# nzw0301/SimCLR

Measured on AMD Instinct MI355X. Metric: pretrain images/sec (whole node) + CIFAR-10 linear-probe top-1, ResNet-50, higher is better.
Workload: dtype bf16

## Files before the change

### simclr_amd/csrc/bindings.cpp

```cpp
#include <ATen/core/Tensor.h>
#include <ATen/ops/empty.h>
#include <ATen/ops/zeros.h>
#include <ATen/hip/HIPContext.h>
#include <c10/util/Exception.h>
#include <torch/library.h>

#include <algorithm>
#include <vector>

#include "kernels.h"

using at::Tensor;

namespace {

hipStream_t cur_stream() { return at::hip::getCurrentHIPStream().stream(); }

void check_dev(const Tensor& t, at::ScalarType dt, const char* name) {
  TORCH_CHECK(t.is_cuda(), name, ": expected a GPU tensor");
  TORCH_CHECK(t.scalar_type() == dt, name, ": expected dtype ", dt, " got ", t.scalar_type());
  TORCH_CHECK(t.is_contiguous(), name, ": expected a contiguous tensor");
}

const uint16_t* bf(const Tensor& t, const char* n) {
// ... 345 lines not shown
  if (a3 != nullptr) {
    TORCH_CHECK(A3->numel() == G.numel() && cf != nullptr && coef->numel() >= 3 * S * CO,
                "conv1x1_bwd_dual: lazy BN-backward needs A3 [M][Co] and coef [3][S][Co]");
  }
  conv1x1_bwd_dual(bf(G, "G"), a3, cf, bf(X, "X"), xs, xm,
                   bf(Wt, "Wt"), bfw(gm, "gm"), f32w(stats, "stats"), f32w(wpart, "wpart"),
                   (int)M, (int)CO, (int)CI, (int)S, (int)bps, cur_stream(), xr, dual8);
}

void conv1x1_bwd_dual_s2_op(const Tensor& G, const c10::optional<Tensor>& A3,
                            const c10::optional<Tensor>& coef, const Tensor& X, const Tensor& Wt,
                            const Tensor& gm, const Tensor& wpart, int64_t S, int64_t bps) {
  TORCH_CHECK(X.dim() == 4 && gm.dim() == 4, "conv1x1_bwd_dual_s2: NHWC 4-D X and gm");
  const int64_t N = X.size(0), H = X.size(1), W = X.size(2), CI = X.size(3);
  const int64_t OH = gm.size(1), OW = gm.size(2);
  TORCH_CHECK(gm.size(0) == N && gm.size(3) == CI && OH == (H + 1) / 2 && OW == (W + 1) / 2,
              "conv1x1_bwd_dual_s2: gm is the stride-2 output map");
  const int64_t Mo = N * OH * OW;
  const int64_t CO = G.numel() / Mo;
  TORCH_CHECK(CO == 512 && CI == 256 && G.numel() == Mo * CO && Wt.numel() == CI * CO,
              "conv1x1_bwd_dual_s2: (Co, Ci) = (512, 256) only");
  TORCH_CHECK(S >= 1 && S <= 2 && N % S == 0 && bps >= 1 && (Mo / S) % (64 * bps) == 0,
              "conv1x1_bwd_dual_s2: every block's rows must lie in one segment");
  TORCH_CHECK(wpart.numel() >= S * bps * CO * CI, "conv1x1_bwd_dual_s2: wpart size");
  TORCH_CHECK(Mo * CO * 2 < (int64_t(1) << 31) && X.numel() * 2 < (int64_t(1) << 31),
              "conv1x1_bwd_dual_s2: 32-bit buffer offsets");
  const uint16_t* a3 = optbf(A3, "A3");
  const float* cf = optf32(coef, "coef");
  TORCH_CHECK(a3 == nullptr && cf == nullptr,
              "conv1x1_bwd_dual_s2: dY must be materialised (no lazy BN-backward form)");
  conv1x1_bwd_dual_s2(bf(G, "G"), a3, cf, bf(X, "X"), bf(Wt, "Wt"), bfw(gm, "gm"),
                      f32w(wpart, "wpart"), (int)Mo, (int)CO, (int)CI, (int)S, (int)bps, (int)H,
                      (int)W, (int)OH, (int)OW, cur_stream());
}

void wgrad_reduce_slabs_op(const Tensor& partial, int64_t splits, const Tensor& out, double beta) {
  const int64_t n = out.numel();
  TORCH_CHECK(n % 4 == 0 && partial.numel() >= splits * n && splits >= 1,
              "wgrad_reduce_slabs: sizes");
  wgrad_reduce_slabs(f32w(partial, "partial"), (int)splits, f32w(out, "out"), (size_t)n,
                     (float)beta, cur_stream());
}

void weight_transform(const Tensor& W, const Tensor& Wt, std::vector<int64_t> p) {
  TORCH_CHECK(p.size() == 10, "weight_transform params");
  const int Co = p[0], KH = p[1], KW = p[2], Ci = p[3], KHs = p[4], KWs = p[5];
  TORCH_CHECK(W.numel() == (int64_t)Co * KH * KW * Ci, "weight_transform: W numel");
  TORCH_CHECK(Wt.numel() == (int64_t)Ci * KHs * KWs * Co, "weight_transform: Wt numel");
  for (int a = 0; a < KHs; ++a) {
    const int kh = (int)p[6] + a * (int)p[7];
    TORCH_CHECK(kh >= 0 && kh < KH, "weight_transform: kh out of range");
  }
  for (int a = 0; a < KWs; ++a) {
    const int kw = (int)p[8] + a * (int)p[9];
    TORCH_CHECK(kw >= 0 && kw < KW, "weight_transform: kw out of range");
  }
  conv_weight_transform(bf(W, "W"), bfw(Wt, "Wt"), Co, KH, KW, Ci, KHs, KWs, p[6], p[7], p[8], p[9],
                        cur_stream());
}

Tensor weight_transform_plan(const std::vector<Tensor>& Ws, const std::vector<Tensor>& Wts,
                             std::vector<int64_t> p) {
  const size_t n = Ws.size();
  TORCH_CHECK(n > 0 && Wts.size() == n && p.size() == 10 * n, "weight_transform_plan sizes");
  Tensor host = at::empty({(int64_t)(n * sizeof(WtDesc) / 8) + 1},
                          at::TensorOptions().dtype(at::kLong));
// ... 853 lines not shown
  m.def("stem_s2d(Tensor img, int creal, int P, Tensor(a!) xs) -> ()", &stem_s2d_op);
  m.def("gemm_sk(Tensor A, Tensor B, Tensor? sc, Tensor? sh, int seg, int KS, Tensor(a!) part, "
        "Tensor? bias, Tensor(b!) out) -> ()", &gemm_sk_op);
  m.def("bn_relu_maxpool(Tensor a, Tensor ss, int S, Tensor(a!) y, Tensor(b!) arg, Tensor(c!) asel, "
        "int K, int Sd, int P) -> ()", &bn_relu_maxpool_op);
  m.def("maxpool_bwd_bn(Tensor gy, Tensor arg, Tensor y, Tensor a, Tensor coef, int S, Tensor(a!) da, "
        "int K, int Sd, int P) -> ()", &maxpool_bwd_bn_op);
  m.def("ce_topk(Tensor logits, Tensor y, float gscale, Tensor(a!) loss, Tensor(b!) rank, Tensor(c!)? dlogits=None) -> ()", &ce_topk_op);
  m.def("class_sums(Tensor X, Tensor y, int NC, Tensor(a!) sums, Tensor(b!) counts) -> ()", &class_sums_op);
  m.def("igemm(Tensor A, Tensor B, Tensor(a!) out, Tensor? bias, Tensor(b!)? stats, int[] geom, Tensor? pro_sc=None, Tensor? pro_sh=None, int pro_seg_rows=0, bool pro_relu=False, int epi_mode=0, Tensor? epi_a=None, Tensor? epi_b=None, int variant=-1, Tensor? epi_ss=None, Tensor? epi_mi=None, int seg_rows=0, int stats_seg_blocks=0, int stats_base=0, Tensor? epi_c=None, Tensor? epi_mask=None, Tensor? epi_c2=None, Tensor? epi_mi2=None, Tensor(c!)? stats2=None, Tensor? pro_d=None, Tensor? A2=None, Tensor? pro_rss=None, Tensor(d!)? pro_out=None, Tensor(e!)? pro_mask=None) -> ()", &igemm);
  m.def("igemm_dual_ok(int v, int[] geom) -> bool", &igemm_dok);
  m.def("igemm_bm(int N) -> int", &igemm_bm);
  m.def("igemm_nvariants() -> int", &igemm_nvariants);
  m.def("igemm_variant_bm(int v) -> int", &igemm_vbm);
  m.def("igemm_variant_bn(int v) -> int", &igemm_vbn);
  m.def("igemm_variant_glds(int v) -> bool", &igemm_vglds);
  m.def("igemm_glds_ok(int[] geom, bool pro, bool bn_bwd_pro) -> bool", &igemm_gldsok);
  m.def("wgrad_nvariants() -> int", &wgrad_nvariants);
  m.def("wgrad_xlin(int mode=-1) -> int", &wgrad_xlin_op);
  m.def("wgrad_variant_glds(int v) -> bool", &wgrad_vglds);
  m.def("igemm_variant_patch(int v) -> bool", [](int64_t v) { return igemm_variant_patch((int)v); });
  m.def("wgrad_variant_area(int v) -> int", [](int64_t v) -> int64_t {
    TORCH_CHECK(v >= 0 && v < wgrad_num_variants(), "wgrad variant out of range");
    return wgrad_variant_area((int)v);
  });
  m.def("igemm_variant_ok(int v, int[] geom, bool pro, bool bn_bwd_pro, int epi_mode=0) -> bool",
        &igemm_vok);
  m.def("wgrad_variant_ok(int v, int[] geom, bool pro, bool dy_pro) -> bool", &wgrad_vok);
  m.def("wgrad_splits(int[] geom, int variant=-1) -> int", &wgrad_nsplit);
  m.def("wgrad_tiles(int[] geom, int variant=-1) -> int", &wgrad_ntiles);
  m.def("conv1x1_bwd_dual_s2(Tensor G, Tensor? A3, Tensor? coef, Tensor X, Tensor Wt, "
        "Tensor(a!) gm, Tensor(b!) wpart, int S, int bps) -> ()", &conv1x1_bwd_dual_s2_op);
  m.def("conv1x1_bwd_dual(Tensor G, Tensor? A3, Tensor? coef, Tensor X, Tensor? xss, Tensor? xmi, Tensor Wt, Tensor(a!) gm, Tensor(b!) stats, Tensor(c!) wpart, int S, int bps, Tensor? Xraw=None, bool dual8=False) -> ()", &conv1x1_bwd_dual_op);
  m.def("wgrad_reduce_slabs(Tensor(a!) partial, int splits, Tensor(b!) out, float beta=0.0) -> ()", &wgrad_reduce_slabs_op);
  m.def("wgrad(Tensor dY, Tensor X, Tensor(a!) partial, Tensor(b!) out, int[] geom, int splits, int creal, float beta, Tensor? pro_sc=None, Tensor? pro_sh=None, int pro_seg_rows=0, bool pro_relu=False, int pro_S=1, int variant=-1, Tensor? dY2=None, Tensor? dp_coef=None, int dp_seg_rows=0, int dp_S=1) -> ()", &wgrad);
  m.def("weight_transform(Tensor W, Tensor(a!) Wt, int[] p) -> ()", &weight_transform);
  m.def("weight_transform_plan(Tensor[] Ws, Tensor[] Wts, int[] p) -> Tensor", &weight_transform_plan);
  m.def("weight_transform_batch(Tensor table, int total_blocks) -> ()", &weight_transform_batch);
  m.def("bn_blocks(int R, int C, int S) -> int", &bn_blocks);
  m.def("bn_stats(Tensor x, int S, Tensor(a!) partial) -> ()", &bn_stats);
  m.def("bn_reduce(Tensor partial, int nblk, int S, int C, Tensor(a!) stats) -> ()", &bn_reduce);
  m.def("bn_finalize(Tensor stats, int S, int C, float count, float eps, float momentum, Tensor(a!)? rm, Tensor(b!)? rv, Tensor(c!) mi, Tensor(d!)? nbt, Tensor? gamma=None, Tensor? beta=None, Tensor(e!)? ss=None) -> ()", &bn_final);
  m.def("ipc_collective(int op, Tensor src, Tensor(a!) dst, Tensor peers, Tensor(b!) arena, int site, Tensor(c!) epoch, Tensor(d!) err, int world, int rank) -> ()", &ipc_collective_op);
  m.def("ipc_coll_blocks() -> int", []() -> int64_t { return IPC_COLL_BLOCKS; });
  m.def("bn_reduce_fused(Tensor partial, int nblk, int S, int C, int mode, Tensor(a!)? stats=None, float count=1.0, float eps=1e-5, float momentum=0.1, Tensor(b!)? rm=None, Tensor(c!)? rv=None, Tensor(d!)? mi=None, Tensor(e!)? nbt=None, Tensor? gamma=None, Tensor? beta=None, Tensor(f!)? ss=None, Tensor(g!)? dgamma=None, Tensor(h!)? dbeta=None, Tensor(i!)? coef=None, int ticket_slot=0, Tensor? ipc_peers=None, Tensor(j!)? ipc_arena=None, int ipc_site=0, Tensor(k!)? ipc_epoch=None, Tensor(l!)? ipc_err=None, int world=1, int rank=0) -> ()", &bn_reduce_fused_op);
  m.def("bn_tickets_init(Tensor like) -> ()", [](const Tensor& like) { (void)tickets_for(like, 0, 0); });
  m.def("bn_apply_ss(Tensor x, Tensor ss, Tensor? res, Tensor? rss, Tensor(a!) y, int S, bool relu, Tensor(b!)? mask=None) -> ()", &bn_apply_ss_op);
  m.def("bn_apply(Tensor x, Tensor? res, Tensor(a!) y, Tensor mi, Tensor? gamma, Tensor? beta, int S, bool relu) -> ()", &bn_apply_op);
  m.def("bn_apply_eval(Tensor x, Tensor? res, Tensor(a!) y, Tensor rm, Tensor rv, Tensor? gamma, Tensor? beta, float eps, bool relu) -> ()", &bn_apply_eval_op);
  m.def("bn_bwd_reduce(Tensor dy, Tensor? y, Tensor x, Tensor mi, int S, bool relu, Tensor(a!) partial) -> ()", &bn_bwd_reduce_op);
  m.def("bn_bwd_finalize(Tensor sums, Tensor mi, Tensor? gamma, int S, int C, float count, Tensor(a!)? dgamma, Tensor(b!)? dbeta, Tensor(c!) coef) -> ()", &bn_bwd_final);
  m.def("bn_bwd_apply(Tensor dy, Tensor? y, Tensor x, Tensor coef, int S, bool relu, Tensor(a!) dx, Tensor(b!)? dres) -> ()", &bn_bwd_apply_op);
  m.def("bn_bwd_apply2(Tensor g, Tensor x1, Tensor coef1, Tensor(a!) dx1, Tensor x2, Tensor coef2, Tensor(b!) dx2, int S) -> ()", &bn_bwd_apply2_op);
  m.def("avgpool_fwd(Tensor x, Tensor(a!) y, int Nb, int HW, int C) -> ()", &avgpool_fwd_op);
  m.def("avgpool_bwd(Tensor dy, Tensor(a!) dx, int Nb, int HW, int C) -> ()", &avgpool_bwd_op);
  m.def("colsum(Tensor x, Tensor(a!) out, float beta) -> ()", &colsum_op);
  m.def("cast_to_bf16(Tensor x, Tensor(a!) y) -> ()", &cast_to_bf16);
  m.def("cast_to_f32(Tensor x, Tensor(a!) y) -> ()", &cast_to_f32);
  m.def("nt_normalize(Tensor z, Tensor(a!) zn, Tensor(b!) inv_norm) -> ()", &nt_normalize);
  m.def("nt_transpose(Tensor x, Tensor(a!) out) -> ()", &nt_transpose);
  m.def("nt_transpose_cols(Tensor x, Tensor(a!) out, int c0) -> ()", &nt_transpose_cols);
  m.def("nt_forward_range(Tensor znT, int R, int col_offset, int n_local, float inv_temp, Tensor(a!) part, int c_lo, int c_hi, int splits, int split_base) -> ()", &nt_forward_range);
  m.def("nt_finish(Tensor part, int R, int splits, Tensor(a!) lse, Tensor(b!) loss) -> ()", &nt_finish);
  m.def("nt_fwd_splits(int R, int C) -> int", &nt_fwd_splits);
  m.def("nt_bwd_splits(int nown, int npart) -> int", &nt_bwd_splits);
  m.def("nt_forward(Tensor znT, int R, int col_offset, int n_local, float inv_temp, Tensor(a!) part, int splits, Tensor(b!) lse, Tensor(c!) loss) -> ()", &nt_forward);
// ... 14 lines not shown
```

### simclr_amd/csrc/conv.hip

```cpp
#include <cstring>
#include "common.h"
#include "kernels.h"

#include <type_traits>
#include <utility>

namespace {

struct IgemmArgs {
  const uint16_t* A;
  const uint16_t* B;
  uint16_t* out;
  const float* bias;
  float* stats;
  int M, N, K;
  int IH, IW, C;
  int OH, OW, KW;
  int ish, isw, dh, dw, ih0, iw0;
  int OHp, OWp, osh, osw, ooh, oow, ldo;
  int direct_out;
  uint32_t a_bytes, b_bytes;
  int nMb, nNb;
  const float* pro_sc;
  const float* pro_sh;
// ... 2869 lines not shown
      for (int i = 0; i < 4; ++i)
        wp[(size_t)(wid * (CO / 8) + fm * 16 + g * 4 + i) * CIT + c0 + fn * 16 + li] =
            accw[fm][fn][i];
  if (PLAIN) return;
#pragma unroll
  for (int off = 1; off < 16; off <<= 1)
#pragma unroll
    for (int fn = 0; fn < NF; ++fn)
#pragma unroll
      for (int r = 0; r < 4; ++r) {
        s1[fn][r] += __shfl_xor(s1[fn][r], off, 64);
        s2[fn][r] += __shfl_xor(s2[fn][r], off, 64);
      }
  if (li == 0) {
#pragma unroll
    for (int fn = 0; fn < NF; ++fn)
#pragma unroll
      for (int r = 0; r < 4; ++r) {
        const int ci = cq * CW + fn * 16 + 4 * g + r;
        red[(rh * CI + ci) * 2 + 0] = s1[fn][r];
        red[(rh * CI + ci) * 2 + 1] = s2[fn][r];
      }
  }
  __syncthreads();
  if (tid < CI) {
    float a = 0.f, b = 0.f;
#pragma unroll
    for (int q = 0; q < RG; ++q) {
      a += red[(q * CI + tid) * 2 + 0];
      b += red[(q * CI + tid) * 2 + 1];
    }
    p.stats[((size_t)blk * 2 + 0) * CIT + c0 + tid] = a;
    p.stats[((size_t)blk * 2 + 1) * CIT + c0 + tid] = b;
  }
}

}

void conv_weight_transform_batch(const WtDesc* d, int n, int total_blocks, hipStream_t s) {
  hipLaunchKernelGGL(weight_transform_batch, dim3(total_blocks), dim3(256), 0, s, d, n);
  HIP_CHECK_LAUNCH();
}

int igemm_num_variants() { return kNumIgemm; }
int igemm_variant_bm(int v) { return IG_VARIANTS[v].bm; }
int igemm_variant_bn(int v) { return IG_VARIANTS[v].bn; }
int igemm_default_variant(int N) { return N <= 64 ? 1 : 0; }
bool igemm_variant_glds(int v) { return v >= 0 && v < kNumIgemm && IG_VARIANTS[v].fam != IG_NT; }
bool igemm_variant_patch(int v) {
  return v >= 0 && v < kNumIgemm && IG_VARIANTS[v].fam == IG_PATCH;
}
bool igemm_glds_ok(const ConvGeom& g, bool pro, bool bn_bwd_pro) {
  if (g.C % 64 != 0) return false;
  return !(pro || bn_bwd_pro) || (g.KH == 1 && g.KW == 1 && g.ih0 == 0 && g.iw0 == 0);
}
static bool direct_out(const ConvGeom& g) {
  return g.osh == 1 && g.osw == 1 && g.ooh == 0 && g.oow == 0 && g.OHp == g.OH && g.OWp == g.OW;
}
bool igemm_patch_ok(const ConvGeom& g) {
  return g.KH == 3 && g.KW == 3 && g.ish == 1 && g.isw == 1 && g.dh == 1 && g.dw == 1 &&
         g.ih0 == -1 && g.iw0 == -1 && g.OH == g.IH && g.OW == g.IW &&
         (g.OW == 16 || g.OW == 32) && (g.C == 64 || g.C == 128) && direct_out(g);
}
static bool glds_doubled_fits(const IgemmVariant& r, const ConvGeom& g, int words) {
  const size_t lds = igemm_glds_pro_offset(r.bm, r.bn, r.threads(), g.C > 64 ? 2 : 1, 2) +
                     (size_t)4 * words * g.C;
// ... 247 lines not shown
  } else if (CO == 256 && CI == 64 && xss == nullptr) {
    hipLaunchKernelGGL((conv1x1_bwd_dual<256, 64, true>), dim3(S * bps), dim3(256), lds, s, a);
  } else if (CO == 256 && CI == 64 && Xraw == nullptr) {
    hipLaunchKernelGGL((conv1x1_bwd_dual<256, 64>), dim3(S * bps), dim3(256), lds, s, a);
  } else {
    fprintf(stderr, "conv1x1_bwd_dual: unsupported Co=%d Ci=%d\n", CO, CI);
    abort();
  }
  HIP_CHECK_LAUNCH();
}

void conv1x1_bwd_dual_s2(const uint16_t* G, const uint16_t* A3, const float* coef,
                         const uint16_t* X, const uint16_t* Wt, uint16_t* gm, float* wpart,
                         int Mo, int CO, int CI, int S, int bps, int H, int W, int OH, int OW,
                         hipStream_t s) {
  Dual1x1Args a{};
  a.G = G; a.A3 = A3; a.coef = coef; a.X = X; a.Wt = Wt; a.gm = gm; a.wpart = wpart;
  a.M = Mo; a.S = S; a.seg_rows = Mo / S; a.bps = bps;
  a.tiles_per_block = a.seg_rows / 32 / bps;
  a.g_bytes = (uint32_t)((size_t)Mo * CO * 2);
  a.x_bytes = (uint32_t)((size_t)(Mo / (OH * OW)) * H * W * CI * 2);
  a.xH = H; a.xW = W; a.xOH = OH; a.xOW = OW;
  if (CO != 512 || CI != 256) {
    fprintf(stderr, "conv1x1_bwd_dual_s2: unsupported Co=%d Ci=%d\n", CO, CI);
    abort();
  }
  const dim3 grid(S * bps * (CI / 64)), blk(512);
  const size_t wl = conv1x1_bwd_dual_w_lds(512);
  hipLaunchKernelGGL((conv1x1_bwd_dual_w<512, 256, false, false, true, true>), grid, blk, wl, s,
                     a);
  HIP_CHECK_LAUNCH();
}

void wgrad_reduce_slabs(float* partial, int splits, float* out, size_t n, float beta,
                        hipStream_t s) {
  reduce_slabs(partial, splits, out, n / 4, beta, true, s);
}
```

### simclr_amd/csrc/kernels.h

```cpp
#pragma once
#include <hip/hip_runtime.h>
#include <stddef.h>
#include <stdint.h>

struct ConvGeom {
  int Nb, IH, IW, C;
  int OH, OW;
  int KH, KW;
  int ish, isw, dh, dw;
  int ih0, iw0;
  int N;
  int OHp, OWp, osh, osw, ooh, oow, ldo;
};

struct ConvFusion {
  const float* pro_sc = nullptr;
  const float* pro_sh = nullptr;
  int pro_seg_rows = 0;
  int pro_relu = 0;
  int pro_S = 1;
  const float* pro_d = nullptr;
  const uint16_t* A2 = nullptr;
  const float* pro_rsc = nullptr;
  const float* pro_rsh = nullptr;
// ... 22 lines not shown
int igemm_num_variants();
int igemm_variant_bm(int v);
int igemm_variant_bn(int v);
int igemm_default_variant(int N);
bool igemm_variant_glds(int v);
bool igemm_variant_patch(int v);
bool igemm_glds_ok(const ConvGeom& g, bool pro, bool bn_bwd_pro);
bool igemm_patch_ok(const ConvGeom& g);
bool igemm_variant_ok(int v, const ConvGeom& g, bool pro, bool bn_bwd_pro, int epi_mode = 0);
bool igemm_dual_ok(int v, const ConvGeom& g);
int igemm_block_m(int N);
void conv_igemm_nt(const ConvGeom& g, const uint16_t* A, size_t a_elems, const uint16_t* B,
                   uint16_t* out, const float* bias, float* stats, const ConvFusion& f,
                   int variant, hipStream_t s);
int wgrad_num_variants();
int wgrad_xlin(int mode);
int wgrad_default_variant(int N);
bool wgrad_variant_glds(int v);
int wgrad_variant_area(int v);
bool wgrad_variant_ok(int v, const ConvGeom& g, bool pro, bool dy_pro);
int wgrad_splits(const ConvGeom& g, int variant);
void conv_wgrad(const ConvGeom& g, const uint16_t* dY, const uint16_t* X, size_t x_elems,
                float* partial, int splits, float* out, int Creal, float beta,
                const ConvFusion& f, int variant, hipStream_t s);
size_t conv1x1_bwd_dual_lds();
void conv1x1_bwd_dual(const uint16_t* G, const uint16_t* A3, const float* coef, const uint16_t* X,
                      const float* xss, const float* xmi, const uint16_t* Wt, uint16_t* gm,
                      float* stats, float* wpart, int M, int CO, int CI, int S, int bps,
                      hipStream_t s, const uint16_t* Xraw = nullptr, bool dual8 = false);
void conv1x1_bwd_dual_s2(const uint16_t* G, const uint16_t* A3, const float* coef,
                         const uint16_t* X, const uint16_t* Wt, uint16_t* gm, float* wpart,
                         int Mo, int CO, int CI, int S, int bps, int H, int W, int OH, int OW,
                         hipStream_t s);
void wgrad_reduce_slabs(float* partial, int splits, float* out, size_t n, float beta,
                        hipStream_t s);
int wgrad_tiles(const ConvGeom& g, int variant);
struct WtDesc {
  const uint16_t* W;
  uint16_t* Wt;
  int Co, KH, KW, Ci, KHs, KWs, kh0, sh, kw0, sw, blk0, nblk;
};
static_assert(sizeof(WtDesc) == 64, "WtDesc layout");
void conv_weight_transform_batch(const WtDesc* d, int n, int total_blocks, hipStream_t s);
void conv_weight_transform(const uint16_t* W, uint16_t* Wt, int Co, int KH, int KW, int Ci,
                           int KHs, int KWs, int kh0, int sh, int kw0, int sw, hipStream_t s);

void bn_stats_partial(const uint16_t* x, int R, int C, int S, float* partial, int* nblk_per_seg,
                      hipStream_t s);
int bn_stats_blocks_per_seg(int R, int C, int S);
int bn_reduce_groups(int nblk);
int bn_reduce_direct_rows();
void bn_reduce_partials(const float* partial, int nblk_per_seg, int S, int C, float* stats,
                        float* ws, hipStream_t s);
void bn_finalize(const float* stats, int S, int C, float count, float eps, float momentum,
                 float* running_mean, float* running_var, float* mean_invstd, int64_t* nbt,
                 const float* gamma, const float* beta, float* scale_shift, hipStream_t s);
struct BnReduceFusedParams {
  const float* partial = nullptr;
  int nblk = 0, S = 1, C = 0, mode = 0;
  float* ws = nullptr;
  unsigned* tickets = nullptr;
  float* stats = nullptr;
  float count = 1.f, eps = 1e-5f, momentum = 0.1f;
  float* running_mean = nullptr;
  float* running_var = nullptr;
  float* mi = nullptr;
// ... 178 lines not shown
```

### simclr_amd/models/fused.py

```python
from __future__ import annotations

import os
from dataclasses import dataclass, field
from typing import List, NamedTuple, Optional, Tuple, Union

import torch
import torch.distributed as dist

from ..ops import _ext
from ..ops.conv_hip import (BlockOut, BnApply, BnBackward, Epilogue, Igemm, StatsOut, WgradDY,
                            WgradX, DgradLaunch, dgrad_plan, fwd_geom, run_wgrad, shadow_ohwi,
                            wt_shape)
from ..parallel import state as pstate
from ..parallel.state import site_key


_SKIP_WGRAD = os.environ.get("SIMCLR_SKIP_WGRAD", "0") == "1"
_SKIP_BNRED = os.environ.get("SIMCLR_EXPERIMENT_SKIP_BNREDUCE", "")


def _empty_nhwc(n, h, w, c, dev, dtype=torch.bfloat16):
    return torch.empty((n, h, w, c), device=dev, dtype=dtype)


# ... 208 lines not shown

class _OutGrad(NamedTuple):
    g3: torch.Tensor
    da: torch.Tensor
    lazy: Optional[LazyBN]
    dad: Optional[torch.Tensor]
    ds_dual: Optional[tuple]


class FusedStages:

    BLOCK_OUT_PROLOGUE = True
    STEM_FUSED = os.environ.get("SIMCLR_FUSED_STEM", "1") != "0"

    bnb_prologue = True
    _bnb_max_cin = 128
    lazy_bn1 = False
    mat_expand_min_cin = 128
    lazy_bn3_ds = True
    _lazy_bn3_ds_dual_only = True
    patch_bnb = os.environ.get("SIMCLR_PATCH_BNB", "1") != "0"
    wgrad_stream = os.environ.get("SIMCLR_WGRAD_STREAM", "1") != "0"
    branch_stream = os.environ.get("SIMCLR_BRANCH_STREAM", "1") != "0"
    compact_ds = True
    block_out_min_hw = 1
    block_out_prologue = BLOCK_OUT_PROLOGUE
    fused_bwd1x1 = True
    fused_bwd1x1_wide = True
    dual8 = True
    dual_reduce_main = False
    fused_ds_dual = True
    ds_dual_stream = "main"
    fused_ds_dual_s2 = False
    bwd1x1_bps = _BWD1X1_BPS
    bwd1x1_bps_wide = 64
    stem_s2d = True

    _side = _branch = _wt_event = _s2d_cache = _wt_sig = _wt_table = None
    _wt_ready = False
    stem = _stem_block = stem_pool = None

    def __init__(self, resnet: torch.nn.Module, segments: int = 2):
        from .resnet import BasicBlock, Bottleneck
        self.resnet = resnet
        self.S = segments
        self.calls = 0
        self.dual_launches = 0
        self.out_apply_calls = 0
        self._side_keep: List[torch.Tensor] = []
        self._wt_cache = {}
        self._dual_cache = {}
        self._patch_bnb_cache = {}
        self.block_out_prologue = type(self).BLOCK_OUT_PROLOGUE
        for kv in filter(None, os.environ.get("SIMCLR_FUSED_ATTRS", "").split(",")):
            k, v = kv.split("=", 1)
            if not hasattr(self, k):
                raise ValueError(f"SIMCLR_FUSED_ATTRS: FusedStages has no switch {k!r}")
            if v.lower() in ("true", "false"):
                setattr(self, k, v.lower() == "true")
            else:
                try:
                    setattr(self, k, int(v))
                except ValueError:
                    setattr(self, k, v)
        self.stem_fused = type(self).STEM_FUSED
        from .resnet import _Identity
        from ..ops.pooling import MaxPool2d
        mp = getattr(resnet, "maxpool", None)
# ... 144 lines not shown

    def _bn_bwd(self, ops, bn, partial, nblk_seg: int, bs: _BNState, S: int, st) -> torch.Tensor:
        return self._bn_bwd_finish(ops, self._bn_bwd_start(ops, bn, partial, nblk_seg, bs, S, st),
                                   S)

    def _memo(self, name: str) -> dict:
        if name not in vars(self):
            setattr(self, name, {})
        return vars(self)[name]

    def _side_stream(self, dev) -> "torch.cuda.Stream":
        if self._side is None or self._side.device != dev:
            self._side = torch.cuda.Stream(device=dev)
        return self._side

    def _issue_wgrad(self, cs: _ConvSpec, keep, compute, main: bool = False) -> None:
        if _SKIP_WGRAD:
            compute = lambda out: None
        side = self._side if self.wgrad_stream and not main else None
        if side is None:
            _deliver_grad(cs.conv.weight, compute)
            return
        self._side_keep.extend(keep)
        side.wait_stream(torch.cuda.current_stream(keep[0].device))
        with torch.cuda.stream(side):
            _deliver_grad(cs.conv.weight, compute)

    def _reduce_slabs(self, ops, cs: _ConvSpec, wpart: torch.Tensor, nslab: int) -> None:
        self._issue_wgrad(cs, (wpart,), lambda out: ops.wgrad_reduce_slabs(wpart, nslab, out),
                          main=self.dual_reduce_main)

    def _wgrad(self, ops, dyn, xn, cs: _ConvSpec, pro_ss: Optional[torch.Tensor], S: int,
               bnb: Optional[LazyBN] = None, main: bool = False):
        Nb, H, W, C = xn.shape
        Co = cs.conv.out_channels
        OH, OW = dyn.shape[1], dyn.shape[2]
        s2d = pro_ss is None and self._s2d_ok(cs, xn)
        if s2d:
            xn = self._s2d_input(ops, xn)
            g = fwd_geom(Nb, xn.shape[1], xn.shape[2], 16, OH, OW, 4, 4, 1, 0, Co)
        else:
            g = fwd_geom(Nb, H, W, C, OH, OW, cs.k, cs.k, cs.stride, cs.pad, Co)
        M = Nb * OH * OW
        pro = WgradX(pro_ss[0], pro_ss[1], M // S, True, S) if pro_ss is not None else None
        dpro = WgradDY(*bnb, M // S, S) if bnb is not None else None

        concurrent = bool(self.wgrad_stream) and self._side is not None and not main

        def compute(out):
            if s2d:
                gs = torch.empty((Co, 4, 4, 16), device=dyn.device, dtype=torch.float32)
                run_wgrad(ops, dyn, xn, gs, g, 16, pro=pro, dpro=dpro, concurrent=concurrent)
                self._s2d_unfold_grad(gs, out)
            else:
                run_wgrad(ops, dyn, xn, out, g, cs.conv.in_channels, pro=pro, dpro=dpro,
                          concurrent=concurrent)

        self._issue_wgrad(cs, [t for t in (dyn, xn, pro_ss, *(bnb or ())) if t is not None],
                          compute, main)

    @staticmethod
    def _bwd1x1_bps(rows_seg: int, cap: int = _BWD1X1_BPS) -> int:
        tiles = rows_seg // 64
        b = min(cap, tiles)
        while b > 1 and tiles % b:
            b -= 1
# ... 89 lines not shown
        return cs.k == 1 and cout >= 4 * cin and cin >= self.mat_expand_min_cin

    def _lazy_bn3_ds_ok(self, b: _BlockSpec, tp: _BlockTape, aL: torch.Tensor, S: int) -> bool:
        L = len(b.convs) - 1
        if not (self.lazy_bn3_ds and L > 0 and self._bnb_ok(b.convs[L], aL, S)):
            return False
        if not self._lazy_bn3_ds_dual_only:
            return True
        xin, pro_ss = tp.ins[L]
        return self._bwd1x1_ok(b.convs[L], aL, xin, pro_ss, tp.acts[L - 1], S)

    def _patch_bnb_ok(self, ops, cs: _ConvSpec, a: torch.Tensor, S: int) -> bool:
        if not (self.patch_bnb and a.is_cuda and cs.k == 3 and cs.stride == 1 and cs.pad == 1):
            return False
        Nb, H, W, C = a.shape
        M = Nb * H * W
        if M % S or (M // S) % 256:
            return False
        Ci = cs.conv.in_channels
        key = (Nb, H, W, C, Ci)
        cache = self._memo("_patch_bnb_cache")
        if key not in cache:
            g = dgrad_plan(Nb, H, W, Ci, H, W, C, 3, 1, 1).launches[0].geom
            cache[key] = any(ops.igemm_variant_patch(v) and ops.igemm_variant_ok(v, g, True, True)
                             for v in range(ops.igemm_nvariants()))
        return cache[key]

    def _lazy_bn1_ok(self, b: _BlockSpec, a1: torch.Tensor, S: int) -> bool:
        cs0 = b.convs[0]
        M = a1.numel() // a1.shape[-1]
        return (self.lazy_bn1 and cs0.k == 1 and cs0.stride == 1
                and M % S == 0 and (M // S) % 256 == 0)

    def _dgrad(self, ops, dyn, cs: _ConvSpec, in_shape, S: int, accumulate: bool = False,
               dx: Optional[torch.Tensor] = None,
               bn_epi: Union[None, MaskEpi, ResEpi] = None, bnb: Optional[LazyBN] = None,
               compact: bool = False, sub_resid: bool = False,
               bnb_out: Optional[torch.Tensor] = None):
        Nb, H, W, Ci = in_shape
        _, OH, OW, Co = dyn.shape
        dev = dyn.device
        if bn_epi is not None:
            bn_epi = (MaskEpi if bn_epi[0] == "mask" else ResEpi)._make(bn_epi)
        w = shadow_ohwi(cs.conv.weight, Ci)
        plan = dgrad_plan(Nb, H, W, Ci, OH, OW, Co, cs.k, cs.stride, cs.pad, compact)
        launches = [(self._dgrad_weight(ops, cs, w, ln), ln) for ln in plan.launches]
        if compact:
            assert bn_epi is None and not accumulate
            dc = _empty_nhwc(Nb, OH, OW, Ci, dev)
            (wt, ln), = launches
            job = Igemm(dyn, wt, dc, ln.geom)
            job.launch(ops, job.choose(ops))
            return dc, None, 0
        resid_c = None
        if sub_resid:
            assert cs.stride == 1 and (accumulate or bn_epi is not None)
            resid_c = dx if bn_epi is None else bn_epi.resid
            dx = None
        if dx is None:
            dx = _empty_nhwc(Nb, H, W, Ci, dev)
        if plan.zero_fill:
            assert bn_epi is None, "BN-epilogue dgrad needs every output position covered"
            if not accumulate:
                dx.zero_()
        if bn_epi is None:
            epi = Epilogue(1, dx) if accumulate else None
            if resid_c is not None:
                epi = Epilogue(1, resid_c, sub=True)
            for wt, ln in launches:
                job = Igemm(dyn, wt, dx, ln.geom, epi=epi)
                job.launch(ops, job.choose(ops))
            return dx, None, 0
        assert not accumulate
        if bn_epi.kind == "mask":
            bs = bn_epi.bs
            epi = Epilogue(3, b=bn_epi.a_prev, ss=bs.ss.view(-1), mi=bs.mi)
# ... 356 lines not shown
    def _chain_bwd(self, ops, st, S, b: _BlockSpec, tp: _BlockTape, o: _OutGrad, prev):
        L = len(b.convs) - 1
        g3, da, lazy = o.g3, o.da, o.lazy
        lazy0 = None
        pend = None
        for i in range(L, 0, -1):
            cs = b.convs[i]
            xin, pro_ss = tp.ins[i]
            a_prev, bs_prev = tp.acts[i - 1], tp.bns[i - 1]
            _ext.TAG = f"{b.name} conv{i + 1} dgrad"
            dyn, bnb = (g3, lazy) if (i == L and lazy is not None) else (da, None)
            if pend is not None:
                gsrc, lazy_b = pend
                pend = None
                dy_m = torch.empty_like(lazy_b.a)
                gm, part, nb = self._dgrad(ops, gsrc, cs, a_prev.shape, S,
                                           bn_epi=MaskEpi("mask", a_prev, bs_prev),
                                           bnb=lazy_b, bnb_out=dy_m)
                wdy, wbnb = dy_m, None
            elif self._bwd1x1_ok(cs, dyn, xin, pro_ss, a_prev, S):
                _ext.TAG = f"{b.name} conv{i + 1} dgrad+wgrad"
                gm, part, nb = self._bwd1x1_fused(ops, dyn, bnb, cs, a_prev, bs_prev, S, xin)
                wdy = None
            else:
                gm, part, nb = self._dgrad(ops, dyn, cs, a_prev.shape, S,
                                           bn_epi=MaskEpi("mask", a_prev, bs_prev), bnb=bnb)
                wdy, wbnb = dyn, bnb
            h = self._bn_bwd_start(ops, b.convs[i - 1].bn, part, nb, bs_prev, S, st)
            if wdy is not None:
                _ext.TAG = f"{b.name} conv{i + 1} wgrad"
                self._wgrad(ops, wdy, xin, cs, pro_ss, S, bnb=wbnb)
            _ext.TAG = f"{b.name} bn{i} bwd"
            coef = self._bn_bwd_finish(ops, h, S)
            if i == 1 and prev is not None and self._lazy_bn1_ok(b, a_prev, S):
                lazy0 = LazyBN(a_prev, coef)
                da = gm
                continue
            if i - 1 >= 1 and self._patch_bnb_ok(ops, b.convs[i - 1], a_prev, S):
                pend = (gm, LazyBN(a_prev, coef))
                continue
            da_next = torch.empty_like(a_prev)
            ops.bn_bwd_apply(gm, None, a_prev, coef, S, False, da_next, None)
            da = da_next
        return da, lazy0

    def _conv1_dgrad(self, ops, st, S, b: _BlockSpec, tp: _BlockTape, o: _OutGrad, da, lazy0,
                     resid, join, compact: bool, prev):
        cs0 = b.convs[0]
        if b.down is None:
            resid = o.g3
        elif join is not None:
            torch.cuda.current_stream(tp.ad.device).wait_stream(join)
        elif resid is None:
            _ext.TAG = f"{b.name} ds dgrad"
            resid, _, _ = self._dgrad(ops, o.dad, b.down, tp.x.shape, S, compact=compact)
        _ext.TAG = f"{b.name} conv1 dgrad"
        if prev is None:
            dx, _, _ = self._dgrad(ops, da, cs0, tp.x.shape, S, accumulate=True, dx=resid,
                                   sub_resid=compact)
            return dx, None
        pb, ptp = prev
        pds = pb.down is not None
        dx, part, nb = self._dgrad(ops, da, cs0, tp.x.shape, S, bnb=lazy0,
                                   dx=resid if b.down is not None and not compact else None,
                                   sub_resid=compact,
                                   bn_epi=ResEpi("res", resid, ptp.mask, ptp.acts[-1],
                                                 ptp.bns[-1].mi, ptp.ad if pds else None,
# ... 36 lines not shown
```

Baseline: 24830.

## Fuse conv1 BN-backward, dgrad, wgrad and next BN stats into one kernel

Adds a fused kernel for the first 1x1 conv of non-downsampling bottleneck blocks. It applies the lazy BN-backward to dY, computes dgrad and wgrad partials from the same LDS tile, and in its epilogue adds the residual, applies the ReLU mask and accumulates the previous BN's backward statistics (optionally for two BN streams). The Python side routes conv1 dgrad to it and defers the wgrad to a slab reduction. This removes several separate passes over dY, X and the residual, at the cost of a large single-occupancy kernel with heavy LDS use.

```diff
diff --git a/simclr_amd/csrc/bindings.cpp b/simclr_amd/csrc/bindings.cpp
--- a/simclr_amd/csrc/bindings.cpp
+++ b/simclr_amd/csrc/bindings.cpp
@@ -401,6 +401,58 @@
   conv1x1_bwd_dual_s2(bf(G, "G"), a3, cf, bf(X, "X"), bf(Wt, "Wt"), bfw(gm, "gm"),
                       f32w(wpart, "wpart"), (int)Mo, (int)CO, (int)CI, (int)S, (int)bps, (int)H,
                       (int)W, (int)OH, (int)OW, cur_stream());
+}
+
+void conv1_bwd_dual_op(const Tensor& G, const Tensor& A1, const Tensor& coef, const Tensor& X,
+                       const Tensor& Wt, const Tensor& res, const Tensor& mask, const Tensor& c1,
+                       const Tensor& mi1, const c10::optional<Tensor>& c2,
+                       const c10::optional<Tensor>& mi2, const Tensor& gm, const Tensor& stats,
+                       const c10::optional<Tensor>& stats2, const Tensor& wpart, int64_t S,
+                       int64_t bps) {
+  const int64_t CI = gm.size(-1);
+  const int64_t M = gm.numel() / CI;
+  TORCH_CHECK(M > 0 && G.numel() % M == 0, "conv1_bwd_dual: G rows");
+  const int64_t CO = G.numel() / M;
+  TORCH_CHECK((CO == 64 || CO == 128) && (CI == 256 || CI == 512),
+              "conv1_bwd_dual: Co 64 | 128 and Ci 256 | 512");
+  const int64_t bmt = conv1_bwd_dual_tile((int)CO);
+  TORCH_CHECK(S >= 1 && bps >= 1 && M % S == 0 && (M / S) % 64 == 0 &&
+                  (M / S) % (bmt * bps) == 0,
+              "conv1_bwd_dual: whole 64-row tiles per segment, equal tile shares per block");
+  TORCH_CHECK(A1.numel() == M * CO && X.numel() == M * CI && Wt.numel() == CI * CO &&
+                  res.numel() == M * CI && c1.numel() == M * CI,
+              "conv1_bwd_dual: operand sizes");
+  TORCH_CHECK(coef.numel() >= 3 * S * CO && mi1.numel() >= 2 * S * CI,
+              "conv1_bwd_dual: coef [3][S][Co], mi [2][S][Ci]");
+  check_dev(mask, at::kByte, "mask");
+  TORCH_CHECK(mask.numel() * 8 >= M * CI, "conv1_bwd_dual: mask size");
+  TORCH_CHECK(stats.numel() >= S * bps * 2 * CI && wpart.numel() >= S * bps * CO * CI,
+              "conv1_bwd_dual: stats / wpart size");
+  TORCH_CHECK(M * CI * 2 < (int64_t(1) << 31), "conv1_bwd_dual: 32-bit buffer offsets");
+  const uint16_t* c2p = optbf(c2, "c2");
+  const float* mi2p = optf32(mi2, "mi2");
+  float* st2 = optf32w(stats2, "stats2");
+  TORCH_CHECK((c2p != nullptr) == (mi2p != nullptr) && (c2p != nullptr) == (st2 != nullptr),
+              "conv1_bwd_dual: c2, mi2 and stats2 together");
+  if (c2p != nullptr)
+    TORCH_CHECK(c2->numel() == M * CI && mi2->numel() >= 2 * S * CI &&
+                    stats2->numel() >= S * bps * 2 * CI,
+                "conv1_bwd_dual: second BN stream sizes");
+  TORCH_CHECK(gm.data_ptr() != X.data_ptr() && gm.data_ptr() != c1.data_ptr() &&
+                  (c2p == nullptr || gm.data_ptr() != c2->data_ptr()),
+              "conv1_bwd_dual: gm must not alias X or the x-hat sources");
+  conv1_bwd_dual(bf(G, "G"), bf(A1, "A1"), f32(coef, "coef"), bf(X, "X"), bf(Wt, "Wt"),
+                 bf(res, "res"), mask.data_ptr<uint8_t>(), bf(c1, "c1"), f32(mi1, "mi1"), c2p,
+                 mi2p, bfw(gm, "gm"), f32w(stats, "stats"), st2, f32w(wpart, "wpart"), (int)M,
+                 (int)CO, (int)CI, (int)S, (int)bps, cur_stream());
+}
+
+bool conv1_bwd_dual_ok_op(std::vector<int64_t> gv, int64_t S) {
+  TORCH_CHECK(gv.size() == 22, "conv geometry must have 22 entries");
+  ConvGeom g;
+  int* p = &g.Nb;
+  for (int i = 0; i < 22; ++i) p[i] = (int)gv[i];
+  return conv1_bwd_dual_ok(g, (int)S);
 }
 
 void wgrad_reduce_slabs_op(const Tensor& partial, int64_t splits, const Tensor& out, double beta) {
@@ -1320,6 +1372,13 @@
   m.def("conv1x1_bwd_dual_s2(Tensor G, Tensor? A3, Tensor? coef, Tensor X, Tensor Wt, "
         "Tensor(a!) gm, Tensor(b!) wpart, int S, int bps) -> ()", &conv1x1_bwd_dual_s2_op);
   m.def("conv1x1_bwd_dual(Tensor G, Tensor? A3, Tensor? coef, Tensor X, Tensor? xss, Tensor? xmi, Tensor Wt, Tensor(a!) gm, Tensor(b!) stats, Tensor(c!) wpart, int S, int bps, Tensor? Xraw=None, bool dual8=False) -> ()", &conv1x1_bwd_dual_op);
+  m.def("conv1_bwd_dual(Tensor G, Tensor A1, Tensor coef, Tensor X, Tensor Wt, Tensor res, "
+        "Tensor mask, Tensor c1, Tensor mi1, Tensor? c2, Tensor? mi2, Tensor(a!) gm, "
+        "Tensor(b!) stats, Tensor(c!)? stats2, Tensor(d!) wpart, int S, int bps) -> ()",
+        &conv1_bwd_dual_op);
+  m.def("conv1_bwd_dual_ok(int[] geom, int S) -> bool", &conv1_bwd_dual_ok_op);
+  m.def("conv1_bwd_dual_tile(int Co) -> int",
+        [](int64_t co) -> int64_t { return conv1_bwd_dual_tile((int)co); });
   m.def("wgrad_reduce_slabs(Tensor(a!) partial, int splits, Tensor(b!) out, float beta=0.0) -> ()", &wgrad_reduce_slabs_op);
   m.def("wgrad(Tensor dY, Tensor X, Tensor(a!) partial, Tensor(b!) out, int[] geom, int splits, int creal, float beta, Tensor? pro_sc=None, Tensor? pro_sh=None, int pro_seg_rows=0, bool pro_relu=False, int pro_S=1, int variant=-1, Tensor? dY2=None, Tensor? dp_coef=None, int dp_seg_rows=0, int dp_S=1) -> ()", &wgrad);
   m.def("weight_transform(Tensor W, Tensor(a!) Wt, int[] p) -> ()", &weight_transform);
diff --git a/simclr_amd/csrc/conv.hip b/simclr_amd/csrc/conv.hip
--- a/simclr_amd/csrc/conv.hip
+++ b/simclr_amd/csrc/conv.hip
@@ -2925,6 +2925,262 @@
     }
     p.stats[((size_t)blk * 2 + 0) * CIT + c0 + tid] = a;
     p.stats[((size_t)blk * 2 + 1) * CIT + c0 + tid] = b;
+  }
+}
+
+struct Conv1DualArgs {
+  const uint16_t* G;
+  const uint16_t* A1;
+  const float* coef;
+  const uint16_t* X;
+  const uint16_t* Wt;
+  const uint16_t* res;
+  const uint8_t* mask;
+  const uint16_t* c1;
+  const float* mi1;
+  const uint16_t* c2;
+  const float* mi2;
+  uint16_t* gm;
+  float* stats;
+  float* stats2;
+  float* wpart;
+  int S, seg_rows, bps, tiles_per_block;
+  uint32_t g_bytes, x_bytes;
+};
+
+constexpr int conv1_dual_tile(int CO, bool two = false) { return CO == 64 && !two ? 64 : 32; }
+
+template <int CO>
+__device__ __forceinline__ int conv1_wkey(int r) {
+  if constexpr (CO == 64)
+    return ((r >> 1) & 1) | (((r >> 3) & 1) << 1) | (((r >> 4) & 1) << 2);
+  else
+    return (r & 3) | (((r >> 3) & 3) << 2);
+}
+
+template <int CO, int CIT, bool TWO>
+__global__ __launch_bounds__(512, 1) void conv1_bwd_dual(Conv1DualArgs p) {
+  constexpr int BMT = conv1_dual_tile(CO, TWO);
+  constexpr int CI = 256;
+  constexpr int NH = CIT / CI, NT = 512;
+  constexpr int RF = BMT / 16;
+  constexpr int WM = 2, WN = 4;
+  constexpr int TCO = CO / WM, TKK = CI / WN;
+  static_assert((CO == 64 || CO == 128) && CIT % CI == 0, "conv1 dual tile mappings");
+  static_assert(BMT * (CO / 8) <= NT, "at most one dY chunk per thread and tile");
+  extern __shared__ __attribute__((aligned(16))) char smem[];
+  uint16_t* Ds = (uint16_t*)smem;
+  uint16_t* Xs = Ds + 2 * BMT * CO;
+  uint16_t* Ws = Xs + 2 * BMT * CI;
+  float* Tb = (float*)(Ws + CI * CO);
+  float* Cf = Tb + 4 * CI;
+
+  const int tid = threadIdx.x, lane = tid & 63;
+  const int wid = __builtin_amdgcn_readfirstlane(tid >> 6);
+  const int g = lane >> 4, li = lane & 15;
+  const int lb = xcd_remap(blockIdx.x, gridDim.x);
+  const int half = lb % NH;
+  const int blk = lb / NH;
+  const int c0 = half * CI;
+  const int seg = blk / p.bps;
+  const int mbeg = seg * p.seg_rows + (blk - seg * p.bps) * p.tiles_per_block * BMT;
+  const int T = p.tiles_per_block;
+
+  const __amdgpu_buffer_rsrc_t rg = buf_rsrc(p.G, p.g_bytes);
+  const __amdgpu_buffer_rsrc_t ra = buf_rsrc(p.A1, p.g_bytes);
+  const __amdgpu_buffer_rsrc_t rx = buf_rsrc(p.X, p.x_bytes);
+
+  for (int c = tid; c < CI * CO / 8; c += NT) {
+    const int row = c / (CO / 8), ch = c % (CO / 8);
+    *(u32x4*)(Ws + row * CO + ((ch ^ conv1_wkey<CO>(row)) * 8)) =
+        *(const u32x4*)(p.Wt + ((size_t)(c0 + row) * CO + ch * 8));
+  }
+  for (int i = tid; i < (TWO ? 4 : 2) * CI; i += NT) {
+    const int k = i / CI, c = i % CI;
+    Tb[i] = (k < 2 ? p.mi1 : p.mi2)[((k & 1) * p.S + seg) * CIT + c0 + c];
+  }
+  for (int i = tid; i < 3 * CO; i += NT) {
+    const int k = i / CO, c = i % CO;
+    Cf[i] = p.coef[(k * p.S + seg) * CO + c];
+  }
+
+  constexpr int GCH = CO / 8, XCH = CI / 8;
+  constexpr int XR = NT / XCH;
+  constexpr int XJ = BMT / XR;
+  const int gch = tid % GCH, grow = tid / GCH;
+  const bool gown = BMT * GCH == NT || wid < BMT * GCH / 64;
+  const int xch = tid % XCH, xrow = tid / XCH;
+
+  u32x4 rG[2], rA[2], rX[2][XJ];
+  auto gload = [&](int t, u32x4& G1, u32x4& A1, u32x4 (&X4)[XJ]) {
+    const int m0 = mbeg + t * BMT;
+    const uint32_t off = (uint32_t)(((size_t)(m0 + grow) * CO + gch * 8) * 2);
+    if (gown) {
+      G1 = __builtin_amdgcn_raw_buffer_load_b128(rg, off, 0, 0);
+      A1 = __builtin_amdgcn_raw_buffer_load_b128(ra, off, 0, 0);
+    }
+#pragma unroll
+    for (int j = 0; j < XJ; ++j)
+      X4[j] = __builtin_amdgcn_raw_buffer_load_b128(
+          rx, (uint32_t)(((size_t)(m0 + xrow + XR * j) * CIT + c0 + xch * 8) * 2), 0, 0);
+  };
+  auto lstore = [&](int buf, const u32x4& G1, const u32x4& A1, const u32x4 (&X4)[XJ]) {
+    if (gown)
+      *(u32x4*)(Ds + buf * BMT * CO + grow * CO + tr_swz<CO>(grow, gch * 8)) =
+          bnbwd8(G1, A1, Cf + gch * 8, Cf + CO + gch * 8, Cf + 2 * CO + gch * 8, true);
+#pragma unroll
+    for (int j = 0; j < XJ; ++j) {
+      const int r = xrow + XR * j;
+      *(u32x4*)(Xs + buf * BMT * CI + r * CI + tr_swz<CI>(r, xch * 8)) = X4[j];
+    }
+  };
+
+  struct Epi {
+    u32x4 ea[RF], ec[RF], ec2[RF];
+    unsigned bits[RF];
+  };
+  const int ecol = wid * 32 + 8 * g;
+  auto eload = [&](int t, Epi& e) {
+#pragma unroll
+    for (int rf = 0; rf < RF; ++rf) {
+      const size_t o = (size_t)(mbeg + t * BMT + rf * 16 + li) * CIT + c0 + ecol;
+      e.ea[rf] = __builtin_nontemporal_load((const u32x4*)(p.res + o));
+      e.ec[rf] = __builtin_nontemporal_load((const u32x4*)(p.c1 + o));
+      if (TWO) e.ec2[rf] = *(const u32x4*)(p.c2 + o);
+      e.bits[rf] = p.mask[o >> 3];
+    }
+  };
+
+  f32x4 accw[TCO / 16][TKK / 16];
+#pragma unroll
+  for (int i = 0; i < TCO / 16; ++i)
+#pragma unroll
+    for (int j = 0; j < TKK / 16; ++j) accw[i][j] = (f32x4){0.f, 0.f, 0.f, 0.f};
+  float s1[8], s2[8], s3[8];
+#pragma unroll
+  for (int e = 0; e < 8; ++e) { s1[e] = 0.f; s2[e] = 0.f; s3[e] = 0.f; }
+
+  auto compute = [&](int t, const Epi& ep) {
+    const int cur = t & 1;
+    const uint16_t* Db = Ds + cur * BMT * CO;
+    f32x4 accd[RF][2];
+#pragma unroll
+    for (int rf = 0; rf < RF; ++rf)
+#pragma unroll
+      for (int h = 0; h < 2; ++h) accd[rf][h] = (f32x4){0.f, 0.f, 0.f, 0.f};
+#pragma unroll
+    for (int ks = 0; ks < CO / 32; ++ks) {
+      const int lch = ks * 4 + g;
+      bf16x8 af[2];
+#pragma unroll
+      for (int h = 0; h < 2; ++h) {
+        const int wr = wid * 32 + 8 * (li >> 2) + 4 * h + (li & 3);
+        af[h] = *(const bf16x8*)(Ws + wr * CO + ((lch ^ conv1_wkey<CO>(wr)) * 8));
+      }
+#pragma unroll
+      for (int rf = 0; rf < RF; ++rf) {
+        const int mrow = rf * 16 + li;
+        const bf16x8 bfr = *(const bf16x8*)(Db + mrow * CO + tr_swz<CO>(mrow, lch * 8));
+#pragma unroll
+        for (int h = 0; h < 2; ++h)
+          accd[rf][h] = __builtin_amdgcn_mfma_f32_16x16x32_bf16(af[h], bfr, accd[rf][h], 0, 0, 0);
+      }
+    }
+    wgrad_mma<CO, CI, WM, WN, BMT / 32>(Db, Xs + cur * BMT * CI, accw);
+    float mu[8], in[8], mu2[8], in2[8];
+#pragma unroll
+    for (int e = 0; e < 8; ++e) {
+      mu[e] = Tb[ecol + e];
+      in[e] = Tb[CI + ecol + e];
+      if (TWO) {
+        mu2[e] = Tb[2 * CI + ecol + e];
+        in2[e] = Tb[3 * CI + ecol + e];
+      }
+    }
+#pragma unroll
+    for (int rf = 0; rf < RF; ++rf) {
+      const size_t o = (size_t)(mbeg + t * BMT + rf * 16 + li) * CIT + c0 + ecol;
+      const unsigned bits = ep.bits[rf];
+      u32x4 w;
+#pragma unroll
+      for (int e = 0; e < 4; ++e) {
+        const f32x4& a = accd[rf][e >> 1];
+        const uint32_t dx = pack2bf(a[2 * (e & 1)], a[2 * (e & 1) + 1]);
+        const uint32_t sum =
+            pack2bf(lo_bf(dx) + lo_bf(ep.ea[rf][e]), hi_bf(dx) + hi_bf(ep.ea[rf][e]));
+        const float g0 = (bits >> (2 * e)) & 1u ? lo_bf(sum) : 0.f;
+        const float g1 = (bits >> (2 * e + 1)) & 1u ? hi_bf(sum) : 0.f;
+        w[e] = pack2bf(g0, g1);
+        s1[2 * e] += g0;
+        s2[2 * e] += g0 * ((lo_bf(ep.ec[rf][e]) - mu[2 * e]) * in[2 * e]);
+        s1[2 * e + 1] += g1;
+        s2[2 * e + 1] += g1 * ((hi_bf(ep.ec[rf][e]) - mu[2 * e + 1]) * in[2 * e + 1]);
+        if (TWO) {
+          s3[2 * e] += g0 * ((lo_bf(ep.ec2[rf][e]) - mu2[2 * e]) * in2[2 * e]);
+          s3[2 * e + 1] += g1 * ((hi_bf(ep.ec2[rf][e]) - mu2[2 * e + 1]) * in2[2 * e + 1]);
+        }
+      }
+      __builtin_nontemporal_store(w, (u32x4*)(p.gm + o));
+    }
+  };
+
+  __syncthreads();
+  if (T > 0) {
+    gload(0, rG[0], rA[0], rX[0]);
+    lstore(0, rG[0], rA[0], rX[0]);
+  }
+  if (T > 1) gload(1, rG[1], rA[1], rX[1]);
+  __syncthreads();
+  for (int t = 0; t < T; t += 2) {
+    {
+      Epi ep;
+      eload(t, ep);
+      if (t + 2 < T) gload(t + 2, rG[0], rA[0], rX[0]);
+      compute(t, ep);
+    }
+    if (t + 1 < T) lstore(1, rG[1], rA[1], rX[1]);
+    asm volatile("s_waitcnt lgkmcnt(0)" ::: "memory");
+    __builtin_amdgcn_s_barrier();
+    if (t + 1 >= T) break;
+    {
+      Epi ep;
+      eload(t + 1, ep);
+      if (t + 3 < T) gload(t + 3, rG[1], rA[1], rX[1]);
+      compute(t + 1, ep);
+    }
+    if (t + 2 < T) lstore(0, rG[0], rA[0], rX[0]);
+    asm volatile("s_waitcnt lgkmcnt(0)" ::: "memory");
+    __builtin_amdgcn_s_barrier();
+  }
+  float* wp = p.wpart + (size_t)blk * CO * CIT;
+  const int wm = wid / WN, wn = wid % WN;
+#pragma unroll
+  for (int fm = 0; fm < TCO / 16; ++fm)
+#pragma unroll
+    for (int fn = 0; fn < TKK / 16; ++fn)
+#pragma unroll
+      for (int i = 0; i < 4; ++i)
+        wp[(size_t)(wm * TCO + fm * 16 + g * 4 + i) * CIT + c0 + wn * TKK + fn * 16 + li] =
+            accw[fm][fn][i];
+#pragma unroll
+  for (int off = 1; off < 16; off <<= 1)
+#pragma unroll
+    for (int e = 0; e < 8; ++e) {
+      s1[e] += __shfl_xor(s1[e], off, 64);
+      s2[e] += __shfl_xor(s2[e], off, 64);
+      if (TWO) s3[e] += __shfl_xor(s3[e], off, 64);
+    }
+  if (li == 0) {
+#pragma unroll
+    for (int e = 0; e < 8; ++e) {
+      const size_t c = (size_t)c0 + ecol + e;
+      p.stats[((size_t)blk * 2 + 0) * CIT + c] = s1[e];
+      p.stats[((size_t)blk * 2 + 1) * CIT + c] = s2[e];
+      if (TWO) {
+        p.stats2[((size_t)blk * 2 + 0) * CIT + c] = s1[e];
+        p.stats2[((size_t)blk * 2 + 1) * CIT + c] = s3[e];
+      }
+    }
   }
 }
 
@@ -3238,6 +3494,55 @@
   HIP_CHECK_LAUNCH();
 }
 
+int conv1_bwd_dual_tile(int CO) { return conv1_dual_tile(CO); }
+
+bool conv1_bwd_dual_ok(const ConvGeom& g, int S) {
+  if (!(g.KH == 1 && g.KW == 1 && g.ish == 1 && g.isw == 1 && g.ih0 == 0 && g.iw0 == 0 &&
+        g.OH == g.IH && g.OW == g.IW && direct_out(g)))
+    return false;
+  if (!(g.N == 64 || g.N == 128) || !(g.C == 256 || g.C == 512) || g.C % 64 != 0) return false;
+  if (g.ldo != g.N) return false;
+  const long long M = (long long)g.Nb * g.OH * g.OW;
+  if (S < 1 || M % S != 0 || (M / S) % 64 != 0) return false;
+  return M * g.C * 2 < (1LL << 31);
+}
+
+template <int CO, int CIT>
+static void launch_conv1_dual(const Conv1DualArgs& a, int blocks, hipStream_t s) {
+  const int BMT = conv1_dual_tile(CO, a.c2 != nullptr);
+  const size_t lds = (size_t)2 * BMT * CO * 2 + (size_t)2 * BMT * 256 * 2 + (size_t)256 * CO * 2 +
+                     (size_t)4 * 256 * 4 + (size_t)3 * CO * 4;
+  const dim3 grid(blocks * (CIT / 256)), blk(512);
+  if (a.c2 != nullptr)
+    hipLaunchKernelGGL((conv1_bwd_dual<CO, CIT, true>), grid, blk, lds, s, a);
+  else
+    hipLaunchKernelGGL((conv1_bwd_dual<CO, CIT, false>), grid, blk, lds, s, a);
+}
+
+void conv1_bwd_dual(const uint16_t* G, const uint16_t* A1, const float* coef, const uint16_t* X,
+                    const uint16_t* Wt, const uint16_t* res, const uint8_t* mask,
+                    const uint16_t* c1, const float* mi1, const uint16_t* c2, const float* mi2,
+                    uint16_t* gm, float* stats, float* stats2, float* wpart, int M, int CO,
+                    int CI, int S, int bps, hipStream_t s) {
+  Conv1DualArgs a{};
+  a.G = G; a.A1 = A1; a.coef = coef; a.X = X; a.Wt = Wt; a.res = res; a.mask = mask;
+  a.c1 = c1; a.mi1 = mi1; a.c2 = c2; a.mi2 = mi2; a.gm = gm;
+  a.stats = stats; a.stats2 = stats2; a.wpart = wpart;
+  a.S = S; a.seg_rows = M / S; a.bps = bps;
+  a.tiles_per_block = a.seg_rows / conv1_dual_tile(CO, c2 != nullptr) / bps;
+  a.g_bytes = (uint32_t)((size_t)M * CO * 2);
+  a.x_bytes = (uint32_t)((size_t)M * CI * 2);
+  if (CO == 64 && CI == 256) launch_conv1_dual<64, 256>(a, S * bps, s);
+  else if (CO == 128 && CI == 256) launch_conv1_dual<128, 256>(a, S * bps, s);
+  else if (CO == 64 && CI == 512) launch_conv1_dual<64, 512>(a, S * bps, s);
+  else if (CO == 128 && CI == 512) launch_conv1_dual<128, 512>(a, S * bps, s);
+  else {
+    fprintf(stderr, "conv1_bwd_dual: unsupported Co=%d Ci=%d\n", CO, CI);
+    abort();
+  }
+  HIP_CHECK_LAUNCH();
+}
+
 void wgrad_reduce_slabs(float* partial, int splits, float* out, size_t n, float beta,
                         hipStream_t s) {
   reduce_slabs(partial, splits, out, n / 4, beta, true, s);
diff --git a/simclr_amd/csrc/kernels.h b/simclr_amd/csrc/kernels.h
--- a/simclr_amd/csrc/kernels.h
+++ b/simclr_amd/csrc/kernels.h
@@ -78,6 +78,13 @@
                          const uint16_t* X, const uint16_t* Wt, uint16_t* gm, float* wpart,
                          int Mo, int CO, int CI, int S, int bps, int H, int W, int OH, int OW,
                          hipStream_t s);
+bool conv1_bwd_dual_ok(const ConvGeom& g, int S);
+int conv1_bwd_dual_tile(int CO);
+void conv1_bwd_dual(const uint16_t* G, const uint16_t* A1, const float* coef, const uint16_t* X,
+                    const uint16_t* Wt, const uint16_t* res, const uint8_t* mask,
+                    const uint16_t* c1, const float* mi1, const uint16_t* c2, const float* mi2,
+                    uint16_t* gm, float* stats, float* stats2, float* wpart, int M, int CO,
+                    int CI, int S, int bps, hipStream_t s);
 void wgrad_reduce_slabs(float* partial, int splits, float* out, size_t n, float beta,
                         hipStream_t s);
 int wgrad_tiles(const ConvGeom& g, int variant);
diff --git a/simclr_amd/models/fused.py b/simclr_amd/models/fused.py
--- a/simclr_amd/models/fused.py
+++ b/simclr_amd/models/fused.py
@@ -264,8 +264,12 @@
     fused_ds_dual = True
     ds_dual_stream = "main"
     fused_ds_dual_s2 = False
+    fused_conv1_dual = True
+    fused_conv1_dual_wide = True
     bwd1x1_bps = _BWD1X1_BPS
     bwd1x1_bps_wide = 64
+    conv1_dual_bps = _BWD1X1_BPS
+    conv1_dual_bps_wide = 64
     stem_s2d = True
 
     _side = _branch = _wt_event = _s2d_cache = _wt_sig = _wt_table = None
@@ -476,6 +480,10 @@
 
     def _wgrad(self, ops, dyn, xn, cs: _ConvSpec, pro_ss: Optional[torch.Tensor], S: int,
                bnb: Optional[LazyBN] = None, main: bool = False):
+        slabs = self._memo("_conv1_slabs").pop(id(cs.conv), None)
+        if slabs is not None:
+            self._reduce_slabs(ops, cs, *slabs)
+            return
         Nb, H, W, C = xn.shape
         Co = cs.conv.out_channels
         OH, OW = dyn.shape[1], dyn.shape[2]
@@ -631,6 +639,47 @@
         return (self.lazy_bn1 and cs0.k == 1 and cs0.stride == 1
                 and M % S == 0 and (M // S) % 256 == 0)
 
+    def _conv1_dual_ok(self, ops, b: _BlockSpec, tp: _BlockTape, S: int, prev) -> bool:
+        cs0 = b.convs[0]
+        if (prev is None or b.down is not None or len(b.convs) < 3 or not tp.x.is_cuda
+                or prev[1].mask is None
+                or not (cs0.k == 1 and cs0.stride == 1 and cs0.pad == 0)):
+            return False
+        co, ci = cs0.conv.out_channels, cs0.conv.in_channels
+        if not ((co, ci) == (64, 256) and self.fused_conv1_dual
+                or (co, ci) == (128, 512) and self.fused_conv1_dual_wide):
+            return False
+        Nb, H, W, C = tp.x.shape
+        key = (Nb, H, W, C, co, S)
+        cache = self._memo("_conv1_dual_cache")
+        if key not in cache:
+            cache[key] = bool(ops.conv1_bwd_dual_ok(
+                fwd_geom(Nb, H, W, C, H, W, 1, 1, 1, 0, co), S))
+        return cache[key]
+
+    def _conv1_dual(self, ops, g1, cs0: _ConvSpec, x, S: int, epi: ResEpi, lazy0: LazyBN):
+        Nb, H, W, Ci = x.shape
+        Co = cs0.conv.out_channels
+        M = Nb * H * W
+        dev = g1.device
+        a1, coef = lazy0
+        two = epi.ad is not None
+        tiles = (M // S) // int(ops.conv1_bwd_dual_tile(Co))
+        bps = min(self.conv1_dual_bps_wide if Ci > 256 else self.conv1_dual_bps, tiles)
+        while bps > 1 and tiles % bps:
+            bps -= 1
+        wt = self._dgrad_weight1x1(ops, cs0, x.shape, H, W)
+        dx = _empty_nhwc(Nb, H, W, Ci, dev)
+        p3 = torch.empty((S * bps * 2 * Ci,), device=dev, dtype=torch.float32)
+        pd = torch.empty_like(p3) if two else None
+        wpart = torch.empty((S * bps * Co * Ci,), device=dev, dtype=torch.float32)
+        _ext.TAG = _ext.TAG.replace("conv1 dgrad", "conv1 bn+dgrad+wgrad")
+        ops.conv1_bwd_dual(g1, a1, coef, x, wt, epi.resid, epi.mask, epi.a_prev,
+                           epi.mi.view(-1), epi.ad, epi.mid.view(-1) if two else None, dx, p3,
+                           pd, wpart, S, bps)
+        self._memo("_conv1_slabs")[id(cs0.conv)] = (wpart, S * bps)
+        return dx, ((p3, pd) if two else p3), bps
+
     def _dgrad(self, ops, dyn, cs: _ConvSpec, in_shape, S: int, accumulate: bool = False,
                dx: Optional[torch.Tensor] = None,
                bn_epi: Union[None, MaskEpi, ResEpi] = None, bnb: Optional[LazyBN] = None,
@@ -641,6 +690,11 @@
         dev = dyn.device
         if bn_epi is not None:
             bn_epi = (MaskEpi if bn_epi[0] == "mask" else ResEpi)._make(bn_epi)
+        xin = self._memo("_conv1_x").pop(id(cs.conv), None)
+        if xin is not None:
+            assert (bnb is not None and bn_epi is not None and bn_epi.kind == "res" and dx is None
+                    and bnb_out is None and not (accumulate or compact or sub_resid))
+            return self._conv1_dual(ops, dyn, cs, xin, S, bn_epi, bnb)
         w = shadow_ohwi(cs.conv.weight, Ci)
         plan = dgrad_plan(Nb, H, W, Ci, OH, OW, Co, cs.k, cs.stride, cs.pad, compact)
         launches = [(self._dgrad_weight(ops, cs, w, ln), ln) for ln in plan.launches]
@@ -1063,7 +1117,10 @@
                 self._wgrad(ops, wdy, xin, cs, pro_ss, S, bnb=wbnb)
             _ext.TAG = f"{b.name} bn{i} bwd"
             coef = self._bn_bwd_finish(ops, h, S)
-            if i == 1 and prev is not None and self._lazy_bn1_ok(b, a_prev, S):
+            fuse1 = i == 1 and self._conv1_dual_ok(ops, b, tp, S, prev)
+            if i == 1 and prev is not None and (fuse1 or self._lazy_bn1_ok(b, a_prev, S)):
+                if fuse1:
+                    self._memo("_conv1_x")[id(b.convs[0].conv)] = tp.x
                 lazy0 = LazyBN(a_prev, coef)
                 da = gm
                 continue
```

After: 25050, median of 6. No clear change (+0.9%).
